# albertz/ParseOggVorbis

Measured on AMD Instinct MI355X. Metric: audio packets/sec (blocksize 2048, stereo), higher is better.
Workload: dtype f32; 1 GPU; config3: 65536 stereo packets, blocksize 2048, 64 streams x 1024, floor+coupling+IMDCT+window+overlap-add; packets_per_gpu=65536, parallelism=streams sharded over 1 GPU(s), no data-path collective

## Files before the change

parseoggvorbis_amd/csrc/vorbis_synth_hip.hip:

```cpp
#include <hip/hip_runtime.h>

#include <mutex>
#include <string>

#include <stdlib.h>

#include "vsyn_host.h"
#include "vsyn_device.h"
#include "vsyn_staged.h"
#include "vsyn_prep.h"
#include "vsyn_fused.h"
#include "vsyn_fused_u.h"
#include "vsyn_vq.h"
#include "vsyn_pcm.h"
#include "vsyn_features.h"
#include "vsyn_spectral.h"
#include "vsyn_spectral_lin.h"
#include "vsyn_chroma.h"
#include "vsyn_spectral_post.h"
#include "vsyn_pcen.h"
#include "vsyn_hpss.h"
#include "vsyn_istft.h"
#include "vsyn_effects.h"
#include "vsyn_pv.h"
// ... 378 lines not shown
      fail(err, VSYN_ERR_HIP, "generic fused table upload failed: %s", hipGetErrorString(e));
      return cleanup(VSYN_ERR_HIP);
    }
  }
#undef HC
  *out = h;
  return VSYN_OK;
}

void vsyn_destroy(vsyn_handle* h) {
  if (!h) return;
  (void)hipSetDevice(h->device);
  (void)hipDeviceSynchronize();
  vq_stamps_dump();
  prep_stamps_dump();
  fused_stamps_dump();
  fused_tables_destroy(&h->fused);
  u_tables_destroy(&h->utab);
  if (h->side) (void)hipStreamDestroy(h->side);
  if (h->pre) (void)hipStreamDestroy(h->pre);
  if (h->host_stream) (void)hipStreamDestroy(h->host_stream);
  if (h->ev_join) (void)hipEventDestroy(h->ev_join);
  if (h->ev_self) (void)hipEventDestroy(h->ev_self);
  if (h->ev_reset) (void)hipEventDestroy(h->ev_reset);
  for (uint32_t b = 0; b < vsyn_handle::WS_RING; ++b)
    if (h->ev_pre_done[b]) (void)hipEventDestroy(h->ev_pre_done[b]);
  for (uint32_t b = 0; b < vsyn_handle::EV_RING; ++b)
    if (h->ev_ring[b]) (void)hipEventDestroy(h->ev_ring[b]);
  if (h->d_const) (void)hipFree(h->d_const);
  if (h->d_vq) (void)hipFree(h->d_vq);
  if (h->d_state) (void)hipFree(h->d_state);
  if (h->d_carry) (void)hipFree(h->d_carry);
  if (h->d_status) (void)hipFree(h->d_status);
  for (auto& ev : h->events) {
    (void)hipEventDestroy(ev.first);
    (void)hipEventDestroy(ev.second);
  }
  delete h;
}

uint32_t vsyn_ys_stride(const vsyn_handle* h) { return h ? h->H.ys_stride : 0; }
uint32_t vsyn_channels(const vsyn_handle* h) { return h ? h->H.channels : 0; }
uint32_t vsyn_fused_paths(const vsyn_handle* h) { return h ? (h->fused_mask | (h->vq_tables_in_lds ? 0x100u : 0u)) : 0; }
size_t vsyn_const_block_bytes(const vsyn_handle* h) { return h ? h->host_const.size() : 0; }

int vsyn_profile_enable(vsyn_handle* h, int on) {
  if (!h) return VSYN_ERR_INVALID;
  h->profile = on != 0;
  if (on >= 1 && on <= 3) h->profile_which = on;
  return VSYN_OK;
}

int vsyn_profile_read(vsyn_handle* h, double* mean_ms, uint32_t* launches, const char** kernel_name) {
  if (!h) return VSYN_ERR_INVALID;
  std::lock_guard<std::mutex> lk(h->mu);
  (void)hipSetDevice(h->device);
  double total = 0;
  for (size_t i = 0; i < h->events_used; ++i) {
    (void)hipEventSynchronize(h->events[i].second);
    float ms = 0;
    (void)hipEventElapsedTime(&ms, h->events[i].first, h->events[i].second);
    total += ms;
  }
  if (mean_ms) *mean_ms = h->events_used ? total / (double)h->events_used : 0.0;
  if (launches) *launches = (uint32_t)h->events_used;
  if (kernel_name) *kernel_name = h->profile_kernel;
  h->events_used = 0;
  return VSYN_OK;
}

static hipError_t profile_begin(vsyn_handle* h, hipStream_t s, const char* name) {
  if (!h->profile) return hipSuccess;
  if (h->events_used == h->events.size()) {
    hipEvent_t a, b;
    const unsigned pf = hipEventDisableSystemFence;
    hipError_t e = hipEventCreateWithFlags(&a, pf);
    if (e != hipSuccess) return e;
    e = hipEventCreateWithFlags(&b, pf);
    if (e != hipSuccess) return e;
    h->events.emplace_back(a, b);
  }
  h->profile_kernel = name;
  return hipEventRecord(h->events[h->events_used].first, s);
}
static hipError_t profile_end(vsyn_handle* h, hipStream_t s) {
  if (!h->profile) return hipSuccess;
  hipError_t e = hipEventRecord(h->events[h->events_used].second, s);
  ++h->events_used;
  return e;
}

int vsyn_reset_streams(vsyn_handle* h, void* hip_stream, const char** err) {
  if (!h) return fail(err, VSYN_ERR_INVALID, "handle is NULL");
  std::lock_guard<std::mutex> lk(h->mu);
  HIPCHK(hipSetDevice(h->device));
  HIPCHK(hipMemsetAsync(h->d_state, 0, sizeof(StreamState) * 2 * h->H.max_streams, (hipStream_t)hip_stream));
  HIPCHK(hipEventRecord(h->ev_reset, (hipStream_t)hip_stream));
  h->reset_pending = true;
  return VSYN_OK;
}

int vsyn_sync_status(vsyn_handle* h, void* hip_stream, vsyn_status* status, const char** err) {
  if (!h) return fail(err, VSYN_ERR_INVALID, "handle is NULL");
  HIPCHK(hipSetDevice(h->device));
  HIPCHK(hipStreamSynchronize((hipStream_t)hip_stream));
  DevStatus ds;
  HIPCHK(hipMemcpy(&ds, h->d_status, sizeof(ds), hipMemcpyDeviceToHost));
  if (ds.flags) {
    DevStatus init = {0u, 0xFFFFFFFFu};
    HIPCHK(hipMemcpy(h->d_status, &init, sizeof(init), hipMemcpyHostToDevice));
  }
  if (status) {
    status->flags = ds.flags;
    status->first_bad_packet = ds.first_bad_packet;
  }
  if (ds.flags) return fail(err, VSYN_ERR_STREAM, "device flagged the batch: flags=0x%x first_bad_packet=%u", ds.flags, ds.first_bad_packet);
  return VSYN_OK;
}

static int submit_device_impl(vsyn_handle* h, uint32_t P, const vsyn_packet* d_packets, uint32_t S, const vsyn_segment* d_segments,
                              uint32_t max_seg_packets, const uint16_t* d_ys, const vsyn_vq_batch* d_vq, float* d_residue, float* d_pcm,
                              uint64_t plane_stride, uint32_t* d_emit_len, const vsyn_taps* taps, uint32_t flags, void* hip_stream,
                              const char** err) {
  if (!h) return fail(err, VSYN_ERR_INVALID, "handle is NULL");
  if (P == 0 || S == 0) return VSYN_OK;
  if (!d_packets || !d_segments || !d_ys || !d_residue || !d_pcm) return fail(err, VSYN_ERR_INVALID, "NULL batch pointer");
  if (d_vq) {
    if (!h->d_vq) return fail(err, VSYN_ERR_INVALID, "vsyn_attach_vq has not been called on this handle");
    if (!d_vq->packets || (d_vq->num_cls && !d_vq->cls) || (d_vq->num_entries && !d_vq->entries)) return fail(err, VSYN_ERR_INVALID, "NULL vq batch pointer");
  }
  if (max_seg_packets == 0 || max_seg_packets > P) max_seg_packets = P;
  std::lock_guard<std::mutex> lk(h->mu);
  HIPCHK(hipSetDevice(h->device));
  hipStream_t s = (hipStream_t)hip_stream;
  const ConstHeader& H = h->H;
  const uint32_t C = H.channels;

  const bool want_taps = taps && (taps->after_envelope || taps->pcm_after_mdct);
  const bool use_u = h->u_mixed;
  const uint32_t fmask = h->fused_mask;
  const bool force_staged = want_taps || (flags & VSYN_SUBMIT_STAGED) || !fmask;
  const uint32_t R = force_staged ? std::min<uint32_t>(max_seg_packets, 1024u)
                                  : fused_pick_run_len(h->opt.run_len, (fmask & 1u) || !use_u ? h->fused.waves_per_cu : (int)h->utab.waves_per_cu,
                                                       S, C, max_seg_packets, h->num_cus);
  const uint32_t runs_per_seg = (max_seg_packets + R - 1) / R;

  const bool prep_kernel = !force_staged && (fmask & 2u) && !d_vq && max_seg_packets <= PREP_MAX_SEG_PACKETS && !(flags & VSYN_SUBMIT_PRE_KERNELS);
  hipStream_t ps = !prep_kernel && (flags & VSYN_SUBMIT_INPUTS_READY) && !force_staged ? h->pre : s;
  const uint32_t chunk_packets = max_seg_packets <= LAYOUT_CHUNK_PACKETS ? runs_per_seg * R : (LAYOUT_CHUNK_PACKETS + R - 1u) / R * R;
  const uint32_t chunks_per_seg = (max_seg_packets + chunk_packets - 1u) / chunk_packets;
  const uint32_t prep_nt = std::min<uint32_t>(PREP_THREADS, std::max<uint32_t>(64u, ((max_seg_packets * C + 63u) / 64u) * 64u));
  const uint32_t prep_chunk_runs = std::max<uint32_t>(1u, std::max<uint32_t>(1u, prep_nt / C) / R);
  const uint32_t prep_chunks_per_seg = (runs_per_seg + prep_chunk_runs - 1u) / prep_chunk_runs;
  const uint64_t prep_wgs = (((uint64_t)S * prep_chunks_per_seg + 7u) / 8u) * 16u;
  const bool staged_may_work = force_staged || !(fmask & 2u);
  hipStream_t ss = force_staged ? s : h->side;
  const uint64_t fused_units = (uint64_t)S * runs_per_seg * C;

  if (!prep_kernel && (uint64_t)S * chunks_per_seg > 0x7FFFFFFFull) return fail(err, VSYN_ERR_INVALID, "too many layout chunks");
  if (prep_kernel && prep_wgs > 0x7FFFFFF0ull) return fail(err, VSYN_ERR_INVALID, "too many runs");
  if (!force_staged && fused_units > (use_u ? U_MAX_UNITS : FUSED_MAX_UNITS)) return fail(err, VSYN_ERR_INVALID, "too many runs");
  const uint64_t isub = h->nsub;
  const uint32_t wb = (uint32_t)(isub % vsyn_handle::WS_RING), wb_prev = (uint32_t)((isub + vsyn_handle::WS_RING - 1u) % vsyn_handle::WS_RING);
  HIPCHK(h->ws_info[wb].ensure((size_t)P + 8));
  HIPCHK(h->ws_seg[wb].ensure(S));
  HIPCHK(h->ws_segmap[wb].ensure(P));
  HIPCHK(h->ws_list[wb].ensure(2 * (size_t)P + 64));
  uint16_t* fy = taps && taps->floor_final ? taps->floor_final : nullptr;
  if (!fy) {
    HIPCHK(h->ws_fy[wb].ensure((size_t)P * C * H.ys_stride));
    fy = h->ws_fy[wb].p;
  }
  HIPCHK(h->ws_runcls[wb].ensure((size_t)S * runs_per_seg + 16));
  bool clear_chunks = false;
  if (!prep_kernel && chunks_per_seg > 1 && (size_t)S * chunks_per_seg > h->ws_chunks.cap) {
    HIPCHK(h->ws_chunks.ensure((size_t)S * chunks_per_seg));
    clear_chunks = true;
  }
  float* env = taps && taps->after_envelope ? taps->after_envelope : nullptr;
  float* blk = taps && taps->pcm_after_mdct ? taps->pcm_after_mdct : nullptr;
  if (staged_may_work) {
    const size_t bound = (size_t)P * C * (H.bs[1] / 2);
    if (!env) {
      HIPCHK(h->ws_env.ensure(bound));
      env = h->ws_env.p;
    }
    if (!blk) {
      HIPCHK(h->ws_blk.ensure(2 * bound));
      blk = h->ws_blk.p;
    }
  }
  PktInfo* info = h->ws_info[wb].p;
  SegInfo* sinfo = h->ws_seg[wb].p;
  uint32_t* segmap = h->ws_segmap[wb].p;
  uint32_t* list = h->ws_list[wb].p;

  ++h->nsub;
  uint32_t* cnt = h->ws_count.p + (isub % vsyn_handle::CNT_RING);
  uint32_t* cnt_next = h->ws_count.p + ((isub + 1u) % vsyn_handle::CNT_RING);
  ++h->submit_count;
  const uint32_t epoch = (h->submit_count & 0x3FFFFFFFu) ? h->submit_count : ++h->submit_count;
  if (ps != s) {
    if (isub >= vsyn_handle::WS_RING) {
      const uint64_t need = isub - vsyn_handle::WS_RING;
      const uint32_t slot = (uint32_t)(need % vsyn_handle::EV_RING);
      if (h->ev_ring_submit[slot] == need) {
        HIPCHK(hipStreamWaitEvent(ps, h->ev_ring[slot], 0));
      } else {
        HIPCHK(hipEventRecord(h->ev_self, s));
        HIPCHK(hipStreamWaitEvent(ps, h->ev_self, 0));
      }
    }
    if (h->last_prep_on_main && isub > 0) {
      HIPCHK(hipEventRecord(h->ev_self, s));
      HIPCHK(hipStreamWaitEvent(ps, h->ev_self, 0));
    }
  }
  if (h->pre_done_valid[wb_prev] && h->last_pre_stream != ps) HIPCHK(hipStreamWaitEvent(ps, h->ev_pre_done[wb_prev], 0));
  if (h->reset_pending) HIPCHK(hipStreamWaitEvent(ps, h->ev_reset, 0));

  if (!prep_kernel) {
    if (!h->last_ran_layout) HIPCHK(hipMemsetAsync(h->ws_count.p, 0, sizeof(uint32_t) * vsyn_handle::CNT_RING, ps));
    if (clear_chunks) HIPCHK(hipMemsetAsync(h->ws_chunks.p, 0, h->ws_chunks.cap * sizeof(LayoutChunk), ps));
    const uint32_t lt = std::min(chunk_packets, max_seg_packets) <= LAYOUT_SHORT_PACKETS ? LAYOUT_THREADS_SHORT : LAYOUT_THREADS;
    vsyn_layout_kernel<<<S * chunks_per_seg, lt, layout_lds_bytes(lt, chunk_packets), ps>>>(
        h->d_const, P, d_packets, S, d_segments, plane_stride, info, sinfo, h->d_state, d_emit_len, h->d_status, R, force_staged ? 0u : fmask, list, cnt,
        cnt_next, segmap, h->ws_runcls[wb].p, runs_per_seg, chunk_packets, chunks_per_seg, h->ws_chunks.p, epoch);
    const uint32_t rows = P * C;
    vsyn_floor_unwrap_kernel<<<(rows + UNWRAP_THREADS - 1) / UNWRAP_THREADS, UNWRAP_THREADS, h->unwrap_lds_bytes, ps>>>(h->d_const, P, info, d_ys, fy,
                                                                                                                          h->d_status);
    if (d_vq) {
      if (h->profile_which == 3) HIPCHK(profile_begin(h, ps, "vsyn_residue_vq_kernel"));
      if (h->vq_tables_in_lds)
        vsyn_residue_vq_kernel<true><<<std::min<uint32_t>((P + h->vq_waves - 1u) / h->vq_waves, h->vq_grid), VQ_THREADS * h->vq_waves, h->vq_lds_bytes, ps>>>(
            h->d_const, h->d_vq, P, info, d_vq->packets, d_vq->cls, d_vq->num_cls, d_vq->entries, d_vq->num_entries, d_residue, h->d_status);
      else
        vsyn_residue_vq_kernel<false><<<std::min<uint32_t>(P, h->vq_grid), VQ_THREADS, h->vq_lds_bytes, ps>>>(
            h->d_const, h->d_vq, P, info, d_vq->packets, d_vq->cls, d_vq->num_cls, d_vq->entries, d_vq->num_entries, d_residue, h->d_status);
      if (h->profile_which == 3) HIPCHK(profile_end(h, ps));
    }
  } else {
    PrepCtx pc;
    pc.cb = h->d_const;
    pc.packets = d_packets;
    pc.segs = d_segments;
    pc.ys = d_ys;
    pc.fy = fy;
    pc.info = info;
    pc.sinfo = sinfo;
    pc.state = h->d_state;
    pc.status = h->d_status;
    pc.emit_len = d_emit_len;
    pc.run_cls = h->ws_runcls[wb].p;
    pc.plane_stride = plane_stride;
    pc.long_modes = h->long_modes;
    pc.S = S;
    pc.R = R;
    pc.runs_per_seg = runs_per_seg;
    pc.fused_ok = fmask;
    pc.P = P;
    pc.epoch = epoch;
    pc.chunk_runs = prep_chunk_runs;
    pc.chunks_per_seg = prep_chunks_per_seg;
    vsyn_prep_kernel<<<(uint32_t)prep_wgs, prep_nt, h->prep_lds_bytes, ps>>>(pc);
  }
  if (ps != s) {
    HIPCHK(hipEventRecord(h->ev_pre_done[wb], ps));
    HIPCHK(hipStreamWaitEvent(s, h->ev_pre_done[wb], 0));
  }

  if (staged_may_work) {
    if (!force_staged) {
      if (ps != s) {
        HIPCHK(hipStreamWaitEvent(h->side, h->ev_pre_done[wb], 0));
      } else {
        HIPCHK(hipEventRecord(h->ev_self, s));
        HIPCHK(hipStreamWaitEvent(h->side, h->ev_self, 0));
      }
    }
    const uint32_t grid = force_staged ? std::min<uint32_t>(P * C, 256u * 32u) : 512u;
    vsyn_spectrum_kernel<<<std::min<uint32_t>(grid, P), 256, 0, ss>>>(h->d_const, list, cnt, info, d_residue, fy, env,
                                                                      taps ? taps->floor_curve : nullptr, h->d_status);
    if (force_staged) HIPCHK(profile_begin(h, s, "vsyn_imdct_staged_kernel"));
    vsyn_imdct_staged_kernel<<<grid, 256, (size_t)H.bs[1] * 4, ss>>>(h->d_const, list, cnt, info, env, blk);
    if (force_staged) HIPCHK(profile_end(h, s));
    vsyn_overlap_kernel<<<grid, 256, 0, ss>>>(h->d_const, list, cnt, info, d_segments, sinfo, segmap, blk, d_pcm, plane_stride, h->d_carry);
  }
  if (!force_staged) {
    FusedArgs a;
    a.cb = h->d_const;
    a.binseg = h->fused.d_binseg;
    a.lds_image = h->fused.d_lds;
    a.packets = d_packets;
    a.segs = d_segments;
    a.info = info;
    a.sinfo = sinfo;
    a.run_cls = h->ws_runcls[wb].p;
    a.runs_per_seg = runs_per_seg;
    a.residue = d_residue;
    a.curve = taps ? taps->floor_curve : nullptr;
    a.fy = fy;
    a.pcm = d_pcm;
    a.carry = h->d_carry;
    a.status = h->d_status;
    a.plane_stride = plane_stride;
    a.S = S;
    a.R = R;
    a.fused_ok = use_u ? (fmask & 1u) : fmask;
    a.coupling_mode = (uint32_t)h->fused.coupling_mode;
    if (staged_may_work) HIPCHK(hipEventRecord(h->ev_join, h->side));
    const bool time_u = use_u && (h->profile_which == 2 || !(fmask & 1u));
    hipError_t e = hipSuccess;
    if (a.fused_ok) {
      if (!time_u && (h->profile_which == 1 || h->profile_which == 2)) HIPCHK(profile_begin(h, s, a.curve ? "vsyn_fused_tap_kernel" : fused_kernel_name(H)));
      e = fused_launch(H, h->fused, a, s);
      if (e != hipSuccess) return fail(err, VSYN_ERR_HIP, "fused launch failed: %s", hipGetErrorString(e));
      if (!time_u && (h->profile_which == 1 || h->profile_which == 2)) HIPCHK(profile_end(h, s));
    }
    if (use_u) {
      FusedArgs au = a;
      au.fused_ok = fmask;
      if (time_u && (h->profile_which == 1 || h->profile_which == 2)) HIPCHK(profile_begin(h, s, au.curve ? "vsyn_fused_u_tap_kernel" : "vsyn_fused_u_kernel"));
      e = u_launch(H, h->utab, au, s);
      if (e != hipSuccess) return fail(err, VSYN_ERR_HIP, "generic fused launch failed: %s", hipGetErrorString(e));
      if (time_u && (h->profile_which == 1 || h->profile_which == 2)) HIPCHK(profile_end(h, s));
    }
    if (staged_may_work) HIPCHK(hipStreamWaitEvent(s, h->ev_join, 0));
  }

  h->last_ran_layout = !prep_kernel;
  h->last_prep_on_main = ps == s;
  h->pre_done_valid[wb] = ps != s;
  h->last_pre_stream = ps;
  h->reset_pending = false;
  if (ps != s) {
    const uint32_t slot = (uint32_t)(isub % vsyn_handle::EV_RING);
    HIPCHK(hipEventRecord(h->ev_ring[slot], s));
    h->ev_ring_submit[slot] = isub;
  }
  h->last_S = S;
  h->last_wb = wb;
  HIPCHK(hipGetLastError());
  return VSYN_OK;
}

int vsyn_submit_device(vsyn_handle* h, uint32_t P, const vsyn_packet* d_packets, uint32_t S, const vsyn_segment* d_segments,
                       uint32_t max_seg_packets, const uint16_t* d_ys, const float* d_residue, float* d_pcm,
                       uint64_t plane_stride, uint32_t* d_emit_len, const vsyn_taps* taps, uint32_t flags, void* hip_stream,
                       const char** err) {
  return submit_device_impl(h, P, d_packets, S, d_segments, max_seg_packets, d_ys, nullptr, const_cast<float*>(d_residue), d_pcm, plane_stride,
                            d_emit_len, taps, flags, hip_stream, err);
}

int vsyn_submit_device_vq(vsyn_handle* h, uint32_t P, const vsyn_packet* d_packets, uint32_t S, const vsyn_segment* d_segments,
                          uint32_t max_seg_packets, const uint16_t* d_ys, const vsyn_vq_batch* d_vq, float* d_residue, float* d_pcm,
                          uint64_t plane_stride, uint32_t* d_emit_len, const vsyn_taps* taps, uint32_t flags, void* hip_stream,
                          const char** err) {
  if (!d_vq) return fail(err, VSYN_ERR_INVALID, "vq batch is NULL");
  return submit_device_impl(h, P, d_packets, S, d_segments, max_seg_packets, d_ys, d_vq, d_residue, d_pcm, plane_stride, d_emit_len, taps, flags,
                            hip_stream, err);
}

int vsyn_attach_vq(vsyn_handle* h, const vsyn_vq_setup* vq, const char** err) {
  if (!h) return fail(err, VSYN_ERR_INVALID, "handle is NULL");
  std::vector<uint8_t> block;
  const std::string why = vq_build_block(vq, h->H, block);
  if (!why.empty()) return fail(err, VSYN_ERR_INVALID, "%s", why.c_str());
  std::lock_guard<std::mutex> lk(h->mu);
  HIPCHK(hipSetDevice(h->device));
  const uint32_t lds_budget = 156u * 1024u;
  HIPCHK(hipFuncSetAttribute((const void*)vsyn_residue_vq_kernel<true>, hipFuncAttributeMaxDynamicSharedMemorySize, (int)lds_budget));
  HIPCHK(hipDeviceSynchronize());
  if (h->d_vq) (void)hipFree(h->d_vq);
  h->d_vq = nullptr;
  HIPCHK(hipMalloc((void**)&h->d_vq, block.size()));
  HIPCHK(hipMemcpy(h->d_vq, block.data(), block.size(), hipMemcpyHostToDevice));
  const VqHeader* vh = (const VqHeader*)block.data();
  uint32_t lds_off[7];
  const uint32_t wave_bytes = vq_lds_layout(vh->max_slots, vh->max_classes, lds_off);
  h->vq_tables_in_lds = false;
  h->vq_waves = 1;
  if (vh->img_floats && !h->opt.vq_no_lds_tables) {
    const uint32_t tab_bytes = vq_align16(vh->img_floats * 4u);
    hipFuncAttributes fa;
    HIPCHK(hipFuncGetAttributes(&fa, (const void*)vsyn_residue_vq_kernel<true>));
    const uint32_t regs = ((uint32_t)std::max(fa.numRegs, 1) + 7u) / 8u * 8u;
    const uint32_t cu_waves = 4u * std::min<uint32_t>(8u, 512u / regs);
    uint32_t best_k = 0, best_w = 0;
    for (uint32_t k = 1; k <= 4; ++k) {
      const uint32_t budget = k == 1 ? lds_budget : 128u * 1024u;
      if (budget / k <= tab_bytes + wave_bytes) break;
      const uint32_t w = std::min<uint32_t>({16u, (budget / k - tab_bytes) / wave_bytes, cu_waves / k});
      if (w && k * w > best_k * best_w) best_k = k, best_w = w;
    }
    if (best_w) {
      const uint32_t lds = tab_bytes + best_w * wave_bytes;
      int per_cu = 0;
      HIPCHK(hipOccupancyMaxActiveBlocksPerMultiprocessor(&per_cu, vsyn_residue_vq_kernel<true>, (int)(VQ_THREADS * best_w), lds));
      if (per_cu > 0) {
        h->vq_tables_in_lds = true;
        h->vq_waves = best_w;
        h->vq_lds_bytes = lds;
        h->vq_grid = (uint32_t)h->num_cus * (uint32_t)per_cu;
        if (h->opt.debug) fprintf(stderr, "[vsyn] vq: tables in LDS (%u B), %u waves per workgroup, %d workgroups per CU, %u B LDS\n", tab_bytes, best_w, per_cu, lds);
      }
    }
  }
  if (!h->vq_tables_in_lds) {
    h->vq_lds_bytes = wave_bytes;
    int per_cu = 0;
    HIPCHK(hipOccupancyMaxActiveBlocksPerMultiprocessor(&per_cu, vsyn_residue_vq_kernel<false>, VQ_THREADS, h->vq_lds_bytes));
    h->vq_grid = (uint32_t)h->num_cus * (uint32_t)std::max(per_cu, 1);
  }
  if (h->opt.vq_grid) h->vq_grid = std::min(h->vq_grid, h->opt.vq_grid);
  if (h->opt.debug)
    fprintf(stderr, "[vsyn] vq launch: %u workgroups, %u waves per workgroup, %u B LDS, tables in %s\n", h->vq_grid, h->vq_waves, h->vq_lds_bytes,
// ... 1906 lines not shown
```

parseoggvorbis_amd/csrc/vsyn_prep.h:

```cpp
#pragma once
#include <hip/hip_runtime.h>

#include "vsyn_device.h"
#include "vsyn_floor1.h"
#include "vsyn_staged.h"

#define PREP_MAX_SEG_PACKETS 4096u
#define PREP_WAVES 4
#define PREP_THREADS (PREP_WAVES * 64)

struct PrepCtx {
  const uint8_t* cb;
  const vsyn_packet* packets;
  const vsyn_segment* segs;
  const uint16_t* ys;
  uint16_t* fy;
  PktInfo* info;
  SegInfo* sinfo;
  StreamState* state;
  DevStatus* status;
  uint32_t* emit_len;
  uint8_t* run_cls;
  uint64_t plane_stride, long_modes;
  uint32_t S, R, runs_per_seg, fused_ok, P, epoch;
  uint32_t chunk_runs, chunks_per_seg;
};

#ifdef PREP_STAMPS
#define PREP_NSTAMPS 8
__device__ unsigned long long g_prep_stamps[8192][PREP_NSTAMPS];
#define PSTAMP(i)                                                \
  do {                                                           \
    __builtin_amdgcn_sched_barrier(0);                           \
    const unsigned long long t_ = __builtin_readcyclecounter();  \
    pst_acc[i] += t_ - pst_last;                                 \
    pst_last = t_;                                               \
    __builtin_amdgcn_sched_barrier(0);                           \
  } while (0)
#else
#define PSTAMP(i) do { } while (0)
#endif

__device__ __forceinline__ void prep_wave_scan(AbsScan& inc, uint64_t& rinc, const uint32_t lane) {
#pragma unroll
  for (int d = 1; d < 64; d <<= 1) {
    const AbsScan o = abs_shfl_up(inc, d);
    const uint64_t ro = __shfl_up(rinc, d);
    if ((int)lane >= d) {
      inc = abs_combine(o, inc);
      rinc += ro;
    }
  }
}
__device__ __forceinline__ uint64_t prep_readlane64(uint64_t v, uint32_t l) {
  return (uint64_t)(uint32_t)__builtin_amdgcn_readlane((uint32_t)v, l) | ((uint64_t)(uint32_t)__builtin_amdgcn_readlane((uint32_t)(v >> 32), l) << 32);
}

__device__ __forceinline__ void prep_block_scan(AbsScan& inc, uint64_t& rinc, AbsScan* s_abs, uint64_t* s_res, AbsScan* total, uint64_t* rtotal) {
  const uint32_t lane = threadIdx.x & 63u, wv = threadIdx.x >> 6;
  prep_wave_scan(inc, rinc, lane);
  __syncthreads();
  if (lane == 63u) {
    s_abs[wv] = inc;
    s_res[wv] = rinc;
  }
  __syncthreads();
  AbsScan pre = {0, 0}, tot = {0, 0};
  uint64_t rpre = 0, rtot = 0;
  const uint32_t nw = blockDim.x >> 6;
#pragma unroll
  for (uint32_t w = 0; w < PREP_WAVES; ++w) {
    if (w >= nw) break;
    const AbsScan a = s_abs[w];
    const uint64_t r = s_res[w];
    if (w < wv) {
      pre = abs_combine(pre, a);
      rpre += r;
    }
    tot = abs_combine(tot, a);
    rtot += r;
  }
  inc = abs_combine(pre, inc);
  rinc += rpre;
  *total = tot;
  *rtotal = rtot;
}

__global__ void __launch_bounds__(PREP_THREADS) vsyn_prep_kernel(const PrepCtx A) {
  extern __shared__ __attribute__((aligned(16))) uint32_t s_rows[];
  __shared__ AbsScan s_abs[PREP_WAVES];
  __shared__ uint64_t s_res[PREP_WAVES];
  __shared__ uint32_t s_pk[PREP_THREADS];
  __shared__ uint32_t s_longbits[PREP_MAX_SEG_PACKETS / 32 + 2];
  __shared__ uint32_t s_last_n;
  const uint8_t* __restrict__ cb = A.cb;
  const ConstHeader* H = hdr_of(cb);
  const uint32_t t = threadIdx.x, lane = t & 63u, wave = __builtin_amdgcn_readfirstlane(t >> 6);
  const uint32_t NT = blockDim.x;
  const uint32_t C = H->channels;
  const uint32_t xj = blockIdx.x >> 3;
  const uint32_t role = (xj ^ (xj >> 5)) & 1u, bid = ((xj >> 1) << 3) | (blockIdx.x & 7u);
  const uint32_t g = bid / A.chunks_per_seg, ch = bid % A.chunks_per_seg;
  if (g >= A.S) return;
#ifdef PREP_STAMPS
  unsigned long long pst_acc[PREP_NSTAMPS] = {0, 0, 0, 0, 0, 0, 0, 0};
  unsigned long long pst_last = __builtin_readcyclecounter();
  const unsigned long long pst_t0 = __builtin_amdgcn_s_memrealtime();
#define PSTAMP_FLUSH()                                                                                              \
  do {                                                                                                              \
    const uint32_t unit_ = blockIdx.x * PREP_WAVES + wave;                                                          \
    if (lane == 0 && unit_ < 8192) {                                                                                \
      for (int i_ = 0; i_ < 5; ++i_) g_prep_stamps[unit_][i_] = pst_acc[i_];                                        \
      g_prep_stamps[unit_][5] = pst_t0;                                                                             \
      g_prep_stamps[unit_][6] = __builtin_amdgcn_s_memrealtime();                                                   \
      g_prep_stamps[unit_][7] = 1ull + role;                                                                        \
    }                                                                                                               \
  } while (0)
#else
#define PSTAMP_FLUSH() do { } while (0)
#endif
  const vsyn_segment sg = A.segs[g];
  const uint32_t num = sg.num_packets;
  const uint32_t R = A.R;
  const uint32_t run0 = ch * A.chunk_runs;
  const uint32_t run1 = min(A.runs_per_seg, run0 + A.chunk_runs);
  const uint32_t cs = run0 * R;
  uint8_t* const cls_row = A.run_cls + (size_t)g * A.runs_per_seg;
  if (sg.stream >= H->max_streams || (uint64_t)sg.first_packet + sg.num_packets > A.P || (sg.residue_off & 3)) {
    if (role) return;
    for (uint32_t r = run0 + t; r < run1; r += NT) cls_row[r] = 0xFFu;
    if (ch == 0u && t == 0u) {
      raise_status(A.status, VSYN_ST_BAD_SEGMENT, sg.first_packet < A.P ? sg.first_packet : 0);
      A.sinfo[g] = SegInfo{0, 0, 0, 0};
    }
    return;
  }
  const uint32_t ce = min(num, run1 * R);
  const vsyn_packet* const spk = A.packets + sg.first_packet;
  typedef uint32_t u32x4 __attribute__((ext_vector_type(4)));
  const uint32_t num_modes = H->num_modes, bs0 = H->bs[0], bs1 = H->bs[1];
  const uint64_t long_modes = A.long_modes;
#define PREP_IS_LONG(m) ((m) < num_modes && (m) < 64u && ((long_modes >> (m)) & 1ull))
#define PREP_N_OF_MODE(m) (PREP_IS_LONG(m) ? bs1 : bs0)
  if (role) {
    const uint32_t ce = min(num, run1 * R);
    if (cs >= ce) return;
    const vsyn_packet* const spk = A.packets + sg.first_packet;
    const uint32_t stride = __builtin_amdgcn_readfirstlane(H->ys_stride);
    const MapConst* const maps = (const MapConst*)(cb + H->off_map);
    const uint32_t chan_mask = C >= 32 ? 0xFFFFFFFFu : ((1u << C) - 1u);
    const uint32_t num_modes = H->num_modes;
    const uint32_t ppp = NT / C;
    for (uint32_t base = cs; base < ce; base += ppp) {
      const uint32_t pe = min(ce, base + ppp);
      const uint32_t rp = t / C, c = t - rp * C;
      const bool row_ok = rp < pe - base;
      uint32_t kmode = 0xFFFFFFFFu, fused_mask = 0;
      if (row_ok) {
        typedef uint32_t u32x2 __attribute__((ext_vector_type(2)));
        const u32x2 w = *(const u32x2*)(spk + base + rp);
        kmode = w.x & 0xFFu;
        fused_mask = w.y;
      }
      const bool mode_ok = row_ok && kmode < num_modes;
      uint32_t fl_id = 0xFFFFFFFFu;
      {
        typedef const __attribute__((address_space(4))) uint32_t* kptr;
        uint64_t todo = __ballot(mode_ok);
        while (todo) {
          const uint32_t m = __builtin_amdgcn_readlane(kmode, (uint32_t)__builtin_ctzll(todo));
          const bool mine = mode_ok && kmode == m;
          todo &= ~__ballot(mine);
          const uint32_t mw = *(kptr)(uintptr_t)((const uint8_t*)H->mode_mapping + (m & ~3u));
          const uint32_t mp = (mw >> (8u * (m & 3u))) & 0xFFu;
          if (mine) fl_id = maps[mp].chfloor[c];
        }
      }
      const bool act = mode_ok && (((fused_mask & chan_mask) >> c) & 1u);
      const uint32_t prow = sg.first_packet + base + rp;
      PSTAMP(3);
      floor1_unwrap_rows(A.cb, A.ys, A.fy, A.status, act, fl_id, prow, (size_t)prow * C + c, stride, (floor1_lds_u32*)s_rows + t, NT);
      PSTAMP(4);
    }
    PSTAMP_FLUSH();
    return;
  }
  uint32_t st_slot;
  const StreamState st0 = state_read(A.state, sg.stream, A.epoch, &st_slot);
  const bool reset = (sg.flags & VSYN_SEG_RESET) != 0;
  const uint32_t carry_n = (!reset && st0.has_prev) ? st0.prev_n : 0;
  const int64_t abs0 = reset ? 0 : (int64_t)st0.abs_total_pos;
  SegInfo si;
  si.has_carry = carry_n ? 1u : 0u;
  si.carry_n = carry_n;
  si.parity_in = reset ? 0u : st0.parity;
  si.total_emit = 0;
  if (cs >= num) {
    for (uint32_t r = run0 + t; r < run1; r += NT) cls_row[r] = 0xFFu;
    if (num == 0u && ch == 0u && t == 0u) {
      A.sinfo[g] = si;
      if (reset) state_write(A.state, sg.stream, st_slot, StreamState{0, 0, 0, 0, 0}, A.epoch);
    }
    return;
  }
  PSTAMP(0);

  AbsScan cin = {0, 0};
  uint64_t cres = 0;
  uint32_t prev_n_in = carry_n;
  uint32_t prev_tail_in = carry_n ? st0.prev_tail : 0u;
  bool halo_long = !carry_n;
  if (cs > 0u) {
    const uint32_t per = (cs + NT - 1u) / NT;
    const uint32_t b = min(cs, t * per), e = min(cs, b + per);
    AbsScan agg = {0, 0};
    uint64_t res = 0;
    uint32_t prev_n = 0;
    if (b < e) prev_n = b == 0u ? carry_n : PREP_N_OF_MODE((uint32_t)spk[b - 1u].mode);
    constexpr uint32_t KEEP = 8;
    for (uint32_t base = b; base < e; base += KEEP) {
      u32x4 kq[KEEP];
#pragma unroll
      for (uint32_t j = 0; j < KEEP; ++j)
        if (base + j < e) kq[j] = *(const u32x4*)(spk + base + j);
#pragma unroll
      for (uint32_t j = 0; j < KEEP; ++j)
        if (base + j < e) {
          const uint32_t md = kq[j].x & 0xFFu;
          const uint32_t n = PREP_N_OF_MODE(md);
          const int64_t gran = (int64_t)((uint64_t)kq[j].z | ((uint64_t)kq[j].w << 32));
          agg = abs_combine(agg, abs_element(gran, prev_n ? (int64_t)(prev_n / 4 + n / 4) : 0));
          res += (uint64_t)C * (n / 2);
          prev_n = n;
        }
    }
    prep_block_scan(agg, res, s_abs, s_res, &cin, &cres);
    const uint32_t hm = __builtin_amdgcn_readfirstlane((uint32_t)spk[cs - 1u].mode);
    prev_n_in = PREP_N_OF_MODE(hm);
    halo_long = PREP_IS_LONG(hm);
    prev_tail_in = prev_tail_of(PREP_IS_LONG(hm), (uint8_t)__builtin_amdgcn_readfirstlane((uint32_t)spk[cs - 1u].next_long));
  }
  PSTAMP(1);

  const uint32_t stride = __builtin_amdgcn_readfirstlane(H->ys_stride);
  const MapConst* const maps = (const MapConst*)(cb + H->off_map);
  const uint32_t chan_mask = C >= 32 ? 0xFFFFFFFFu : ((1u << C) - 1u);
  const uint32_t ppp = NT / C;
  for (uint32_t w = t; w < (ce - cs + 1u + 31u) / 32u; w += NT) s_longbits[w] = 0u;
  __syncthreads();
  if (t == 0u && halo_long) s_longbits[0] = 1u;
  for (uint32_t base = cs; base < ce; base += ppp) {
    const uint32_t pe = min(ce, base + ppp);
    const uint32_t q = base + t;
    const bool valid = q < pe;
    vsyn_packet k = {};
    if (valid) {
      const u32x4 w = *(const u32x4*)(spk + q);
      k.mode = (uint8_t)(w.x & 0xFFu);
      k.prev_long = (uint8_t)((w.x >> 8) & 0xFFu);
      k.next_long = (uint8_t)((w.x >> 16) & 0xFFu);
      k.floor_used = w.y;
      k.granule = (int64_t)((uint64_t)w.z | ((uint64_t)w.w << 32));
    }
    const bool mode_ok = valid && k.mode < num_modes;
    const uint32_t kmode = k.mode;
    const uint32_t lng = (valid && PREP_IS_LONG(kmode)) ? 1u : 0u;
    const uint32_t n = lng ? bs1 : bs0;
    __syncthreads();
    const uint32_t tail = prev_tail_of(mode_ok && lng, k.next_long);
    s_pk[t] = n | (tail << 31);
    __syncthreads();
    const uint32_t prev_n = t == 0u ? prev_n_in : (s_pk[t - 1u] & 0x7FFFFFFFu);
    const uint32_t prev_tail = t == 0u ? prev_tail_in : (s_pk[t - 1u] >> 31);
    AbsScan inc = {0, 0};
    uint64_t rinc = 0;
    if (valid) {
      inc = abs_element(k.granule, prev_n ? (int64_t)(prev_n / 4 + n / 4) : 0);
      rinc = (uint64_t)C * (n / 2);
    }
    const AbsScan own_el = inc;
    const uint64_t own_res = rinc;
    AbsScan tot;
    uint64_t rtot;
    prep_block_scan(inc, rinc, s_abs, s_res, &tot, &rtot);
    const uint64_t rex = rinc - own_res;
    AbsScan ex;
    {
      ex = abs_shfl_up(inc, 1);
      if (lane == 0u) {
        AbsScan pre = {0, 0};
        for (uint32_t w = 0; w < wave; ++w) pre = abs_combine(pre, s_abs[w]);
        ex = pre;
      }
    }
    (void)own_el;
    ex = abs_combine(cin, ex);
    const int64_t abs_before = abs_eval(ex, abs0);
    const uint64_t res_off = sg.residue_off + cres + rex;
    const uint32_t p = sg.first_packet + q;
    uint32_t mapping = 0, own = k.floor_used & chan_mask, used = own;
    {
      typedef const __attribute__((address_space(4))) uint32_t* kptr;
      uint64_t todo = __ballot(mode_ok);
      while (todo) {
        const uint32_t m = __builtin_amdgcn_readlane(kmode, (uint32_t)__builtin_ctzll(todo));
        const bool mine = mode_ok && kmode == m;
        todo &= ~__ballot(mine);
        const uint32_t mw = *(kptr)(uintptr_t)((const uint8_t*)H->mode_mapping + (m & ~3u));
        const uint32_t mp = (mw >> (8u * (m & 3u))) & 0xFFu;
        const MapConst* mc = maps + mp;
        const uint32_t ncoup = *(kptr)(uintptr_t)&mc->ncoup;
        uint32_t u = used;
        for (uint32_t i = 0; i < ncoup; ++i) {
          const uint32_t pair = *(kptr)(uintptr_t)&mc->coup[2 * i];
          const uint32_t ma = pair & 0xFFFFu, an = pair >> 16;
          if (((u >> ma) | (u >> an)) & 1u) u |= (1u << ma) | (1u << an);
        }
        if (mine) {
          mapping = mp;
          used = u;
        }
      }
    }
    if (valid) {
      const PktStep ps = pkt_step_core(k, mode_ok, lng, mapping, n, prev_n, prev_tail, abs_before, abs0, res_off, A.plane_stride, own, used);
      if (ps.raise) {
        if (ps.raise & VSYN_ST_BAD_MODE) raise_status(A.status, VSYN_ST_BAD_MODE, p);
        if (ps.raise & VSYN_ST_WINDOW_FLAGS) raise_status(A.status, VSYN_ST_WINDOW_FLAGS, p);
        if (ps.raise & VSYN_ST_GRANULE) raise_status(A.status, VSYN_ST_GRANULE, p);
        if (ps.raise & VSYN_ST_PLANE_OVERFLOW) raise_status(A.status, VSYN_ST_PLANE_OVERFLOW, p);
      }
      A.info[p] = ps.pi;
      if (A.emit_len) A.emit_len[p] = ps.pi.emit;
      if (q == num - 1u) {
        SegInfo so = si;
        so.total_emit = (uint32_t)(ps.abs_after - abs0);
        A.sinfo[g] = so;
        StreamState ns;
        ns.abs_total_pos = (uint64_t)ps.abs_after;
        ns.has_prev = 1;
        ns.prev_n = n;
        ns.prev_tail = tail;
        ns.parity = si.parity_in ^ 1u;
        ns.tag = 0;
        state_write(A.state, sg.stream, st_slot, ns, A.epoch);
      }
      if (mode_ok && lng) atomicOr(&s_longbits[(q - cs + 1u) >> 5], 1u << ((q - cs + 1u) & 31u));
      if (q == pe - 1u) s_last_n = n | (tail << 31);
    }
    __syncthreads();
    PSTAMP(2);
    cin = abs_combine(cin, tot);
    cres += rtot;
    prev_n_in = s_last_n & 0x7FFFFFFFu;
    prev_tail_in = s_last_n >> 31;
  }
  __syncthreads();
  {
    const uint32_t nruns_seg = (num + R - 1u) / R;
    for (uint32_t r = run0 + t; r < run1; r += NT) {
      uint32_t cls = 0xFFu;
      if (r < nruns_seg) {
        const uint32_t first = r * R - cs, end = min(num, (r + 1u) * R) - cs;
        bool all_long = true;
        for (uint32_t w = first >> 5; all_long && w <= (end >> 5); ++w) {
          uint32_t need = 0xFFFFFFFFu;
          if (w == (first >> 5)) need &= 0xFFFFFFFFu << (first & 31u);
          if (w == (end >> 5)) need &= 0xFFFFFFFFu >> (31u - (end & 31u));
          all_long = (s_longbits[w] & need) == need;
        }
        cls = (all_long && (A.fused_ok & 1u)) ? 1u : ((A.fused_ok & 2u) ? 2u : 0u);
      }
      cls_row[r] = (uint8_t)cls;
    }
  }
  PSTAMP_FLUSH();
#undef PREP_IS_LONG
#undef PREP_N_OF_MODE
}

#include <stdio.h>

static inline void prep_stamps_dump() {
#ifdef PREP_STAMPS
  static unsigned long long host[8192][PREP_NSTAMPS];
  if (hipMemcpyFromSymbol(host, HIP_SYMBOL(g_prep_stamps), sizeof(host)) == hipSuccess) {
    unsigned long long t_first = ~0ull;
    for (int u = 0; u < 8192; ++u)
      if (host[u][7] && host[u][5] < t_first) t_first = host[u][5];
    for (unsigned role = 0; role < 2; ++role) {
      double sum[5] = {0}, st = 0, en = 0, en_max = 0, st_max = 0;
      unsigned long long waves = 0;
      for (int u = 0; u < 8192; ++u) {
        if (host[u][7] != 1ull + role) continue;
        ++waves;
        for (int i = 0; i < 5; ++i) sum[i] += (double)host[u][i];
        const double a = (double)(host[u][5] - t_first) / 100.0, b = (double)(host[u][6] - t_first) / 100.0;
        st += a;
        en += b;
        if (a > st_max) st_max = a;
        if (b > en_max) en_max = b;
      }
      if (!waves) continue;
      static const char* nm[5] = {"header + stream state", "scan in front of the chunk", "descriptors, scan, PktInfo", "floor role: descriptors, floor ids", "floor role: chains"};
      fprintf(stderr, "prep stamps, %s role: %llu waves; start %.2f us (latest %.2f), end %.2f us (latest %.2f) after the launch's first wave\n",
              role ? "floor" : "layout", waves, st / waves, st_max, en / waves, en_max);
      for (int i = 0; i < 5; ++i)
        if (sum[i] > 0) fprintf(stderr, "  %-36s %8.0f cycles\n", nm[i], sum[i] / waves);
    }
  }
#endif
}
```

Measured before the change: 273.9 million packets/s.

## Process four packets per thread in prep layout scan and split workgroup roles

The prep kernel's layout role now has each thread handle four consecutive packets. Each thread does a serial local scan before the block-wide scan, and the layout workgroups get their own sizing (lay_nt, span_runs) instead of sharing the interleaved role mapping. Roles are now assigned by contiguous blockIdx ranges, several __syncthreads are dropped, and long-packet bits are set with one masked atomicOr per thread. This cuts the number of scan rounds and barriers per segment, at the cost of more registers and serial work per thread.

```diff
diff --git a/parseoggvorbis_amd/csrc/vorbis_synth_hip.hip b/parseoggvorbis_amd/csrc/vorbis_synth_hip.hip
--- a/parseoggvorbis_amd/csrc/vorbis_synth_hip.hip
+++ b/parseoggvorbis_amd/csrc/vorbis_synth_hip.hip
@@ -554,7 +554,12 @@
   const uint32_t prep_nt = std::min<uint32_t>(PREP_THREADS, std::max<uint32_t>(64u, ((max_seg_packets * C + 63u) / 64u) * 64u));
   const uint32_t prep_chunk_runs = std::max<uint32_t>(1u, std::max<uint32_t>(1u, prep_nt / C) / R);
   const uint32_t prep_chunks_per_seg = (runs_per_seg + prep_chunk_runs - 1u) / prep_chunk_runs;
-  const uint64_t prep_wgs = (((uint64_t)S * prep_chunks_per_seg + 7u) / 8u) * 16u;
+  const uint32_t prep_lay_nt =
+      std::min<uint32_t>(PREP_THREADS, std::max<uint32_t>(64u, (((max_seg_packets + PREP_PPT - 1u) / PREP_PPT + 63u) / 64u) * 64u));
+  const uint32_t prep_span_runs = std::max<uint32_t>(1u, PREP_PPT * prep_lay_nt / R);
+  const uint32_t prep_spans_per_seg = (runs_per_seg + prep_span_runs - 1u) / prep_span_runs;
+  const uint64_t prep_lay_wgs = (uint64_t)S * prep_spans_per_seg;
+  const uint64_t prep_wgs = prep_lay_wgs + (uint64_t)S * prep_chunks_per_seg;
   const bool staged_may_work = force_staged || !(fmask & 2u);
   hipStream_t ss = force_staged ? s : h->side;
   const uint64_t fused_units = (uint64_t)S * runs_per_seg * C;
@@ -664,6 +669,10 @@
     pc.epoch = epoch;
     pc.chunk_runs = prep_chunk_runs;
     pc.chunks_per_seg = prep_chunks_per_seg;
+    pc.span_runs = prep_span_runs;
+    pc.spans_per_seg = prep_spans_per_seg;
+    pc.lay_wgs = (uint32_t)prep_lay_wgs;
+    pc.lay_nt = prep_lay_nt;
     vsyn_prep_kernel<<<(uint32_t)prep_wgs, prep_nt, h->prep_lds_bytes, ps>>>(pc);
   }
   if (ps != s) {
diff --git a/parseoggvorbis_amd/csrc/vsyn_prep.h b/parseoggvorbis_amd/csrc/vsyn_prep.h
--- a/parseoggvorbis_amd/csrc/vsyn_prep.h
+++ b/parseoggvorbis_amd/csrc/vsyn_prep.h
@@ -8,6 +8,7 @@
 #define PREP_MAX_SEG_PACKETS 4096u
 #define PREP_WAVES 4
 #define PREP_THREADS (PREP_WAVES * 64)
+#define PREP_PPT 4u
 
 struct PrepCtx {
   const uint8_t* cb;
@@ -24,6 +25,8 @@
   uint64_t plane_stride, long_modes;
   uint32_t S, R, runs_per_seg, fused_ok, P, epoch;
   uint32_t chunk_runs, chunks_per_seg;
+  uint32_t span_runs, spans_per_seg;
+  uint32_t lay_wgs, lay_nt;
 };
 
 #ifdef PREP_STAMPS
@@ -56,10 +59,10 @@
   return (uint64_t)(uint32_t)__builtin_amdgcn_readlane((uint32_t)v, l) | ((uint64_t)(uint32_t)__builtin_amdgcn_readlane((uint32_t)(v >> 32), l) << 32);
 }
 
-__device__ __forceinline__ void prep_block_scan(AbsScan& inc, uint64_t& rinc, AbsScan* s_abs, uint64_t* s_res, AbsScan* total, uint64_t* rtotal) {
+__device__ __forceinline__ void prep_block_scan(AbsScan& inc, uint64_t& rinc, AbsScan* s_abs, uint64_t* s_res, AbsScan* total, uint64_t* rtotal,
+                                                const uint32_t nw) {
   const uint32_t lane = threadIdx.x & 63u, wv = threadIdx.x >> 6;
   prep_wave_scan(inc, rinc, lane);
-  __syncthreads();
   if (lane == 63u) {
     s_abs[wv] = inc;
     s_res[wv] = rinc;
@@ -67,7 +70,6 @@
   __syncthreads();
   AbsScan pre = {0, 0}, tot = {0, 0};
   uint64_t rpre = 0, rtot = 0;
-  const uint32_t nw = blockDim.x >> 6;
 #pragma unroll
   for (uint32_t w = 0; w < PREP_WAVES; ++w) {
     if (w >= nw) break;
@@ -92,16 +94,16 @@
   __shared__ uint64_t s_res[PREP_WAVES];
   __shared__ uint32_t s_pk[PREP_THREADS];
   __shared__ uint32_t s_longbits[PREP_MAX_SEG_PACKETS / 32 + 2];
-  __shared__ uint32_t s_last_n;
   const uint8_t* __restrict__ cb = A.cb;
   const ConstHeader* H = hdr_of(cb);
   const uint32_t t = threadIdx.x, lane = t & 63u, wave = __builtin_amdgcn_readfirstlane(t >> 6);
-  const uint32_t NT = blockDim.x;
   const uint32_t C = H->channels;
-  const uint32_t xj = blockIdx.x >> 3;
-  const uint32_t role = (xj ^ (xj >> 5)) & 1u, bid = ((xj >> 1) << 3) | (blockIdx.x & 7u);
-  const uint32_t g = bid / A.chunks_per_seg, ch = bid % A.chunks_per_seg;
-  if (g >= A.S) return;
+  const uint32_t role = blockIdx.x >= A.lay_wgs ? 1u : 0u;
+  const uint32_t bid = role ? blockIdx.x - A.lay_wgs : blockIdx.x;
+  const uint32_t per_seg = role ? A.chunks_per_seg : A.spans_per_seg;
+  const uint32_t NT = role ? blockDim.x : A.lay_nt;
+  const uint32_t g = bid / per_seg, ch = bid % per_seg;
+  if (g >= A.S || t >= NT) return;
 #ifdef PREP_STAMPS
   unsigned long long pst_acc[PREP_NSTAMPS] = {0, 0, 0, 0, 0, 0, 0, 0};
   unsigned long long pst_last = __builtin_readcyclecounter();
@@ -122,8 +124,9 @@
   const vsyn_segment sg = A.segs[g];
   const uint32_t num = sg.num_packets;
   const uint32_t R = A.R;
-  const uint32_t run0 = ch * A.chunk_runs;
-  const uint32_t run1 = min(A.runs_per_seg, run0 + A.chunk_runs);
+  const uint32_t wg_runs = role ? A.chunk_runs : A.span_runs;
+  const uint32_t run0 = ch * wg_runs;
+  const uint32_t run1 = min(A.runs_per_seg, run0 + wg_runs);
   const uint32_t cs = run0 * R;
   uint8_t* const cls_row = A.run_cls + (size_t)g * A.runs_per_seg;
   if (sg.stream >= H->max_streams || (uint64_t)sg.first_packet + sg.num_packets > A.P || (sg.residue_off & 3)) {
@@ -205,6 +208,7 @@
   }
   PSTAMP(0);
 
+  const uint32_t nw = NT >> 6;
   AbsScan cin = {0, 0};
   uint64_t cres = 0;
   uint32_t prev_n_in = carry_n;
@@ -234,7 +238,7 @@
           prev_n = n;
         }
     }
-    prep_block_scan(agg, res, s_abs, s_res, &cin, &cres);
+    prep_block_scan(agg, res, s_abs, s_res, &cin, &cres, nw);
     const uint32_t hm = __builtin_amdgcn_readfirstlane((uint32_t)spk[cs - 1u].mode);
     prev_n_in = PREP_N_OF_MODE(hm);
     halo_long = PREP_IS_LONG(hm);
@@ -245,45 +249,59 @@
   const uint32_t stride = __builtin_amdgcn_readfirstlane(H->ys_stride);
   const MapConst* const maps = (const MapConst*)(cb + H->off_map);
   const uint32_t chan_mask = C >= 32 ? 0xFFFFFFFFu : ((1u << C) - 1u);
-  const uint32_t ppp = NT / C;
+  const uint32_t ppp = PREP_PPT * NT;
   for (uint32_t w = t; w < (ce - cs + 1u + 31u) / 32u; w += NT) s_longbits[w] = 0u;
-  __syncthreads();
-  if (t == 0u && halo_long) s_longbits[0] = 1u;
   for (uint32_t base = cs; base < ce; base += ppp) {
     const uint32_t pe = min(ce, base + ppp);
-    const uint32_t q = base + t;
-    const bool valid = q < pe;
-    vsyn_packet k = {};
-    if (valid) {
-      const u32x4 w = *(const u32x4*)(spk + q);
-      k.mode = (uint8_t)(w.x & 0xFFu);
-      k.prev_long = (uint8_t)((w.x >> 8) & 0xFFu);
-      k.next_long = (uint8_t)((w.x >> 16) & 0xFFu);
-      k.floor_used = w.y;
-      k.granule = (int64_t)((uint64_t)w.z | ((uint64_t)w.w << 32));
-    }
-    const bool mode_ok = valid && k.mode < num_modes;
-    const uint32_t kmode = k.mode;
-    const uint32_t lng = (valid && PREP_IS_LONG(kmode)) ? 1u : 0u;
-    const uint32_t n = lng ? bs1 : bs0;
+    const uint32_t q0 = base + PREP_PPT * t;
+    vsyn_packet k[PREP_PPT];
+    bool valid[PREP_PPT], mode_ok[PREP_PPT];
+    uint32_t lng[PREP_PPT], n[PREP_PPT], tail[PREP_PPT];
+    {
+      u32x4 w[PREP_PPT];
+#pragma unroll
+      for (uint32_t j = 0; j < PREP_PPT; ++j) {
+        valid[j] = q0 + j < pe;
+        w[j] = u32x4{0u, 0u, 0u, 0u};
+        if (valid[j]) w[j] = *(const u32x4*)(spk + q0 + j);
+      }
+#pragma unroll
+      for (uint32_t j = 0; j < PREP_PPT; ++j) {
+        k[j].mode = (uint8_t)(w[j].x & 0xFFu);
+        k[j].prev_long = (uint8_t)((w[j].x >> 8) & 0xFFu);
+        k[j].next_long = (uint8_t)((w[j].x >> 16) & 0xFFu);
+        k[j].reserved0 = 0;
+        k[j].floor_used = w[j].y;
+        k[j].granule = (int64_t)((uint64_t)w[j].z | ((uint64_t)w[j].w << 32));
+        const uint32_t kmode = k[j].mode;
+        mode_ok[j] = valid[j] && kmode < num_modes;
+        lng[j] = (valid[j] && PREP_IS_LONG(kmode)) ? 1u : 0u;
+        n[j] = lng[j] ? bs1 : bs0;
+        tail[j] = prev_tail_of(mode_ok[j] && lng[j], k[j].next_long);
+      }
+    }
     __syncthreads();
-    const uint32_t tail = prev_tail_of(mode_ok && lng, k.next_long);
-    s_pk[t] = n | (tail << 31);
+    s_pk[t] = n[PREP_PPT - 1u] | (tail[PREP_PPT - 1u] << 31);
     __syncthreads();
-    const uint32_t prev_n = t == 0u ? prev_n_in : (s_pk[t - 1u] & 0x7FFFFFFFu);
-    const uint32_t prev_tail = t == 0u ? prev_tail_in : (s_pk[t - 1u] >> 31);
+    uint32_t prev_n = t == 0u ? prev_n_in : (s_pk[t - 1u] & 0x7FFFFFFFu);
+    uint32_t prev_tail = t == 0u ? prev_tail_in : (s_pk[t - 1u] >> 31);
+    const uint32_t last_pk = s_pk[NT - 1u];
     AbsScan inc = {0, 0};
     uint64_t rinc = 0;
-    if (valid) {
-      inc = abs_element(k.granule, prev_n ? (int64_t)(prev_n / 4 + n / 4) : 0);
-      rinc = (uint64_t)C * (n / 2);
-    }
-    const AbsScan own_el = inc;
+    {
+      uint32_t pn = prev_n;
+#pragma unroll
+      for (uint32_t j = 0; j < PREP_PPT; ++j)
+        if (valid[j]) {
+          inc = abs_combine(inc, abs_element(k[j].granule, pn ? (int64_t)(pn / 4 + n[j] / 4) : 0));
+          rinc += (uint64_t)C * (n[j] / 2);
+          pn = n[j];
+        }
+    }
     const uint64_t own_res = rinc;
     AbsScan tot;
     uint64_t rtot;
-    prep_block_scan(inc, rinc, s_abs, s_res, &tot, &rtot);
-    const uint64_t rex = rinc - own_res;
+    prep_block_scan(inc, rinc, s_abs, s_res, &tot, &rtot, nw);
     AbsScan ex;
     {
       ex = abs_shfl_up(inc, 1);
@@ -293,67 +311,81 @@
         ex = pre;
       }
     }
-    (void)own_el;
     ex = abs_combine(cin, ex);
-    const int64_t abs_before = abs_eval(ex, abs0);
-    const uint64_t res_off = sg.residue_off + cres + rex;
-    const uint32_t p = sg.first_packet + q;
-    uint32_t mapping = 0, own = k.floor_used & chan_mask, used = own;
+    int64_t abs_before = abs_eval(ex, abs0);
+    uint64_t res_off = sg.residue_off + cres + (rinc - own_res);
+    uint32_t longmask = 0;
+#pragma unroll
+    for (uint32_t j = 0; j < PREP_PPT; ++j) {
+      const uint32_t q = q0 + j, p = sg.first_packet + q;
+      const uint32_t kmode = k[j].mode;
+      uint32_t mapping = 0, own = k[j].floor_used & chan_mask, used = own;
+      {
+        typedef const __attribute__((address_space(4))) uint32_t* kptr;
+        uint64_t todo = __ballot(mode_ok[j]);
+        while (todo) {
+          const uint32_t m = __builtin_amdgcn_readlane(kmode, (uint32_t)__builtin_ctzll(todo));
+          const bool mine = mode_ok[j] && kmode == m;
+          todo &= ~__ballot(mine);
+          const uint32_t mw = *(kptr)(uintptr_t)((const uint8_t*)H->mode_mapping + (m & ~3u));
+          const uint32_t mp = (mw >> (8u * (m & 3u))) & 0xFFu;
+          const MapConst* mc = maps + mp;
+          const uint32_t ncoup = *(kptr)(uintptr_t)&mc->ncoup;
+          uint32_t u = used;
+          for (uint32_t i = 0; i < ncoup; ++i) {
+            const uint32_t pair = *(kptr)(uintptr_t)&mc->coup[2 * i];
+            const uint32_t ma = pair & 0xFFFFu, an = pair >> 16;
+            if (((u >> ma) | (u >> an)) & 1u) u |= (1u << ma) | (1u << an);
+          }
+          if (mine) {
+            mapping = mp;
+            used = u;
+          }
+        }
+      }
+      if (valid[j]) {
+        const PktStep ps = pkt_step_core(k[j], mode_ok[j], lng[j], mapping, n[j], prev_n, prev_tail, abs_before, abs0, res_off, A.plane_stride, own, used);
+        if (ps.raise) {
+          if (ps.raise & VSYN_ST_BAD_MODE) raise_status(A.status, VSYN_ST_BAD_MODE, p);
+          if (ps.raise & VSYN_ST_WINDOW_FLAGS) raise_status(A.status, VSYN_ST_WINDOW_FLAGS, p);
+          if (ps.raise & VSYN_ST_GRANULE) raise_status(A.status, VSYN_ST_GRANULE, p);
+          if (ps.raise & VSYN_ST_PLANE_OVERFLOW) raise_status(A.status, VSYN_ST_PLANE_OVERFLOW, p);
+        }
+        A.info[p] = ps.pi;
+        if (A.emit_len) A.emit_len[p] = ps.pi.emit;
+        if (q == num - 1u) {
+          SegInfo so = si;
+          so.total_emit = (uint32_t)(ps.abs_after - abs0);
+          A.sinfo[g] = so;
+          StreamState ns;
+          ns.abs_total_pos = (uint64_t)ps.abs_after;
+          ns.has_prev = 1;
+          ns.prev_n = n[j];
+          ns.prev_tail = tail[j];
+          ns.parity = si.parity_in ^ 1u;
+          ns.tag = 0;
+          state_write(A.state, sg.stream, st_slot, ns, A.epoch);
+        }
+        if (mode_ok[j] && lng[j]) longmask |= 1u << j;
+        abs_before = ps.abs_after;
+        res_off += (uint64_t)C * (n[j] / 2);
+        prev_n = n[j];
+        prev_tail = tail[j];
+      }
+    }
     {
-      typedef const __attribute__((address_space(4))) uint32_t* kptr;
-      uint64_t todo = __ballot(mode_ok);
-      while (todo) {
-        const uint32_t m = __builtin_amdgcn_readlane(kmode, (uint32_t)__builtin_ctzll(todo));
-        const bool mine = mode_ok && kmode == m;
-        todo &= ~__ballot(mine);
-        const uint32_t mw = *(kptr)(uintptr_t)((const uint8_t*)H->mode_mapping + (m & ~3u));
-        const uint32_t mp = (mw >> (8u * (m & 3u))) & 0xFFu;
-        const MapConst* mc = maps + mp;
-        const uint32_t ncoup = *(kptr)(uintptr_t)&mc->ncoup;
-        uint32_t u = used;
-        for (uint32_t i = 0; i < ncoup; ++i) {
-          const uint32_t pair = *(kptr)(uintptr_t)&mc->coup[2 * i];
-          const uint32_t ma = pair & 0xFFFFu, an = pair >> 16;
-          if (((u >> ma) | (u >> an)) & 1u) u |= (1u << ma) | (1u << an);
-        }
-        if (mine) {
-          mapping = mp;
-          used = u;
-        }
-      }
-    }
-    if (valid) {
-      const PktStep ps = pkt_step_core(k, mode_ok, lng, mapping, n, prev_n, prev_tail, abs_before, abs0, res_off, A.plane_stride, own, used);
-      if (ps.raise) {
-        if (ps.raise & VSYN_ST_BAD_MODE) raise_status(A.status, VSYN_ST_BAD_MODE, p);
-        if (ps.raise & VSYN_ST_WINDOW_FLAGS) raise_status(A.status, VSYN_ST_WINDOW_FLAGS, p);
-        if (ps.raise & VSYN_ST_GRANULE) raise_status(A.status, VSYN_ST_GRANULE, p);
-        if (ps.raise & VSYN_ST_PLANE_OVERFLOW) raise_status(A.status, VSYN_ST_PLANE_OVERFLOW, p);
-      }
-      A.info[p] = ps.pi;
-      if (A.emit_len) A.emit_len[p] = ps.pi.emit;
-      if (q == num - 1u) {
-        SegInfo so = si;
-        so.total_emit = (uint32_t)(ps.abs_after - abs0);
-        A.sinfo[g] = so;
-        StreamState ns;
-        ns.abs_total_pos = (uint64_t)ps.abs_after;
-        ns.has_prev = 1;
-        ns.prev_n = n;
-        ns.prev_tail = tail;
-        ns.parity = si.parity_in ^ 1u;
-        ns.tag = 0;
-        state_write(A.state, sg.stream, st_slot, ns, A.epoch);
-      }
-      if (mode_ok && lng) atomicOr(&s_longbits[(q - cs + 1u) >> 5], 1u << ((q - cs + 1u) & 31u));
-      if (q == pe - 1u) s_last_n = n | (tail << 31);
-    }
-    __syncthreads();
+      const uint32_t b0 = q0 - cs + 1u, sh = b0 & 31u;
+      if (longmask) {
+        atomicOr(&s_longbits[b0 >> 5], longmask << sh);
+        if (sh > 32u - PREP_PPT && (longmask >> (32u - sh))) atomicOr(&s_longbits[(b0 >> 5) + 1u], longmask >> (32u - sh));
+      }
+      if (t == 0u && base == cs && halo_long) atomicOr(&s_longbits[0], 1u);
+    }
     PSTAMP(2);
     cin = abs_combine(cin, tot);
     cres += rtot;
-    prev_n_in = s_last_n & 0x7FFFFFFFu;
-    prev_tail_in = s_last_n >> 31;
+    prev_n_in = last_pk & 0x7FFFFFFFu;
+    prev_tail_in = last_pk >> 31;
   }
   __syncthreads();
   {
```

Measured after the change: 273.6 million packets/s. No clear change (-0.1%).
